# erthward/geonomics

Measured on AMD Instinct MI355X. Metric: individual-timesteps/sec, higher is better.
Workload: dtype u64

## Files before the change

geonomics_amd/csrc/gnx_kernels_demog.hip:

```cpp
#include "gnx_internal.h"
#include <chrono>
#include "gnx_rng.h"
#include "gnx_compact.h"
#include "gnx_half.h"
#include "gnx_xo.h"

#define BIN_BLOCKS 512

__global__ void __launch_bounds__(256)
k_bins(int64_t n, const int32_t* n_dev, const float* x, const float* y, const uint8_t* ghost,
       double inv_hww, int nbx, int nby, int32_t* partials, GnxSetWords sw) {
  extern __shared__ int32_t lds_hist[];
  if (sw.dst && blockIdx.x == 0 && threadIdx.x < 4) sw.dst[threadIdx.x] = sw.v[threadIdx.x];
  if (n_dev) n = *n_dev;
  const int nb = nbx * nby;
  for (int k = threadIdx.x; k < nb; k += blockDim.x) lds_hist[k] = 0;
  __syncthreads();
  const int64_t stride = (int64_t)gridDim.x * blockDim.x;
  for (int64_t i = (int64_t)blockIdx.x * blockDim.x + threadIdx.x; i < n; i += stride) {
    if (ghost && ghost[i]) continue;
    int hx = min(nbx - 1, (int)floor((double)x[i] * inv_hww));
    int hy = min(nby - 1, (int)floor((double)y[i] * inv_hww));
    atomicAdd(&lds_hist[hy * nbx + hx], 1);
  }
  __syncthreads();
  for (int k = threadIdx.x; k < nb; k += blockDim.x) {
    int v = lds_hist[k];
    if (v) atomicAdd(&partials[k], v);
  }
}

__global__ void k_set_words(GnxSetWords sw) {
  if (blockIdx.x == 0 && threadIdx.x < 4) sw.dst[threadIdx.x] = sw.v[threadIdx.x];
}

__global__ void k_bins_global(int64_t n, const float* x, const float* y, const uint8_t* ghost,
                              double inv_hww, int nbx, int nby, int32_t* hist) {
  int64_t i = (int64_t)blockIdx.x * blockDim.x + threadIdx.x;
  if (i >= n) return;
  if (ghost && ghost[i]) return;
  int hx = min(nbx - 1, (int)floor((double)x[i] * inv_hww));
  int hy = min(nby - 1, (int)floor((double)y[i] * inv_hww));
  atomicAdd(&hist[hy * nbx + hx], 1);
}

__global__ void k_nodes(int Jx, int Jy, int nbx, int n_part, const int32_t* partials,
                        const double* areas, double* V) {
  int idx = blockIdx.x * blockDim.x + threadIdx.x;
  if (idx >= Jx * Jy) return;
  int i = idx / Jx, j = idx - i * Jx;
  const int nb = nbx * Jy;
  long long cnt = 0;
  for (int di = -1; di <= 0; ++di)
    for (int dj = -1; dj <= 0; ++dj) {
      int ii = i + di, jj = j + dj;
      if (ii < 0 || jj < 0) continue;
      int b = ii * nbx + jj;
      for (int p = 0; p < n_part; ++p) cnt += partials[(int64_t)p * nb + b];
    }
  V[idx] = (double)cnt / areas[idx];
}

__global__ void k_spline_m(int Jx, int Jy, int along_x, double h, const double* cp,
                           const double* V, double* M) {
// ... 64 lines not shown
  c.hww = h->lat.hww;
  c.inv_hww = 1.0 / h->lat.hww;
  return c;
}

int gnx_l_bins(gnx_state* h, int64_t n, const float* d_x, const float* d_y, const uint8_t* d_ghost,
               int32_t* d_bins, const int32_t* n_dev, const GnxSetWords* sw) {
  const GnxLattice& L = h->lat;
  const int nb = L.nbx * L.nby;
  const int field = (d_bins == h->bins_P) ? 1 : 0;
  if (!h->bins_zeroed[field])
    HIPCHK(hipMemsetAsync(d_bins, 0, (size_t)nb * sizeof(int32_t), h->stream));
  h->bins_zeroed[field] = false;
  if (n > 0) {
    if ((size_t)nb * sizeof(int32_t) <= 48 * 1024) {
      int blocks = (int)std::min<int64_t>(BIN_BLOCKS, std::max<int64_t>(1, (n + 255) / 256));
      hipLaunchKernelGGL(k_bins, dim3(blocks), dim3(256), (size_t)nb * sizeof(int32_t), h->stream,
                         n, n_dev, d_x, d_y, d_ghost, 1.0 / L.hww, L.nbx, L.nby, d_bins,
                         sw ? *sw : GnxSetWords{});
      sw = nullptr;
    } else {
      hipLaunchKernelGGL(k_bins_global, dim3(gnx_grid(n, 256)), dim3(256), 0, h->stream, n, d_x,
                         d_y, d_ghost, 1.0 / L.hww, L.nbx, L.nby, d_bins);
    }
  }
  if (sw)
    hipLaunchKernelGGL(k_set_words, dim3(1), dim3(64), 0, h->stream, *sw);
  HIPCHK(hipGetLastError());
  return 0;
}

__device__ __forceinline__ void spline_line(int J, int64_t base, int64_t stride, double h,
                                            const double* cp, const double* V, double* M) {
  M[base] = 0.0;
  M[base + (int64_t)(J - 1) * stride] = 0.0;
  if (J <= 2) return;
  const double s = 6.0 / (h * h);
  double dprev = 0.0;
  for (int k = 1; k <= J - 2; ++k) {
    double d = s * (V[base + (k - 1) * stride] - 2.0 * V[base + k * stride] +
                    V[base + (k + 1) * stride]);
    double dp = (d - dprev) * cp[k];
    M[base + k * stride] = dp;
    dprev = dp;
  }
  double mnext = dprev;
  for (int k = J - 3; k >= 1; --k) {
    const double m = M[base + k * stride] - cp[k] * mnext;
    M[base + k * stride] = m;
    mnext = m;
  }
}

__device__ __forceinline__ void spline_rows_and_cols(int Jx, int Jy, double hww, const double* cp,
                                                     const double* V, double* Mx, double* My) {
  const int half = blockDim.x / 2;
  if ((int)threadIdx.x < half) {
    for (int line = threadIdx.x; line < Jy; line += half)
      spline_line(Jx, (int64_t)line * Jx, 1, hww, cp, V, Mx);
  } else {
    for (int line = threadIdx.x - half; line < Jx; line += half)
      spline_line(Jy, line, Jx, hww, cp, V, My);
  }
}


__global__ void __launch_bounds__(256)
k_lattice(int Jx, int Jy, int nbx, const int32_t* bins, const double* areas, double hww,
          const double* cp_g, double* C, int32_t* zero_bins, int n_zero,
          unsigned long long* zero_word, int use_lds, int zero_own) {
  extern __shared__ double lat_lds[];
  const int nn = Jx * Jy;
  for (int k = threadIdx.x; k < n_zero; k += blockDim.x) zero_bins[k] = 0;
  if (zero_word && threadIdx.x == 0) *zero_word = 0ull;
  double* W = use_lds ? lat_lds : C;
  double* V = W;
  double* Mx = W + nn;
  double* My = W + 2 * (int64_t)nn;
  double* Mxy = W + 3 * (int64_t)nn;
  const double* cp = cp_g;
  if (use_lds) {
    double* cpl = lat_lds + 4 * (int64_t)nn;
    const int Jm = max(Jx, Jy);
    for (int k = threadIdx.x; k <= Jm; k += blockDim.x) cpl[k] = cp_g[k];
    cp = cpl;
    if (!bins)
      for (int idx = threadIdx.x; idx < nn; idx += blockDim.x) V[idx] = C[idx];
  }
  if (bins) {
    for (int idx = threadIdx.x; idx < nn; idx += blockDim.x) {
      const int i = idx / Jx, j = idx - i * Jx;
      long long cnt = 0;
      for (int di = -1; di <= 0; ++di)
        for (int dj = -1; dj <= 0; ++dj) {
          const int ii = i + di, jj = j + dj;
          if (ii >= 0 && jj >= 0) cnt += bins[ii * nbx + jj];
        }
      V[idx] = (double)cnt / areas[idx];
    }
  }
  __syncthreads();
  if (bins && zero_own)
    for (int k = threadIdx.x; k < nn; k += blockDim.x) const_cast<int32_t*>(bins)[k] = 0;
  spline_rows_and_cols(Jx, Jy, hww, cp, V, Mx, My);
  __syncthreads();
  for (int line = threadIdx.x; line < Jy; line += blockDim.x)
    spline_line(Jx, (int64_t)line * Jx, 1, hww, cp, My, Mxy);
  if (use_lds) {
    __syncthreads();
    for (int idx = threadIdx.x; idx < 4 * nn; idx += blockDim.x) C[idx] = lat_lds[idx];
  }
}

int gnx_l_spline(gnx_state* h, const int32_t* d_bins, GnxSpline* spl,
                 const double* d_nodes_override) {
  return gnx_l_spline_z(h, d_bins, spl, d_nodes_override, false);
}

int gnx_l_spline_z(gnx_state* h, const int32_t* d_bins, GnxSpline* spl,
                   const double* d_nodes_override, bool housekeeping) {
  const GnxLattice& L = h->lat;
  const int64_t nn = (int64_t)L.Jx * L.Jy;
  double* V = spl->c;
  if (d_nodes_override)
    HIPCHK(hipMemcpyAsync(V, d_nodes_override, nn * sizeof(double), hipMemcpyDeviceToDevice,
                          h->stream));
  if (nn <= 65536) {
    int32_t* zb = nullptr;
    int other = -1;
    if (housekeeping && !d_nodes_override) {
      other = (d_bins == h->bins_P) ? 0 : 1;
      zb = other ? h->bins_P : h->bin_partials;
    }
    const size_t lds_bytes = ((size_t)4 * nn + std::max(L.Jx, L.Jy) + 1) * sizeof(double);
    const int use_lds = lds_bytes <= 60 * 1024 ? 1 : 0;
    hipLaunchKernelGGL(k_lattice, dim3(1), dim3(256), use_lds ? lds_bytes : 0, h->stream, L.Jx,
                       L.Jy, L.nbx, d_nodes_override ? nullptr : d_bins, L.areas, L.hww, L.cprime,
                       V, zb, zb ? L.nbx * L.nby : 0,
                       (housekeeping && spl == &h->spl_N) ? h->nmax_bits : nullptr, use_lds, 0);
    if (zb) h->bins_zeroed[other] = true;
    if (housekeeping && spl == &h->spl_N) h->nmax_zeroed = true;
    HIPCHK(hipGetLastError());
    spl->valid = true;
    return 0;
  }
  if (!d_nodes_override)
    hipLaunchKernelGGL(k_nodes, dim3(gnx_grid(nn, 128)), dim3(128), 0, h->stream, L.Jx, L.Jy, L.nbx,
                       1, d_bins, L.areas, V);
  double* Mx = V + nn;
  double* My = V + 2 * nn;
  double* Mxy = V + 3 * nn;
  hipLaunchKernelGGL(k_spline_m, dim3(gnx_grid(L.Jy, 64)), dim3(64), 0, h->stream, L.Jx, L.Jy, 1,
                     L.hww, L.cprime, V, Mx);
  hipLaunchKernelGGL(k_spline_m, dim3(gnx_grid(L.Jx, 64)), dim3(64), 0, h->stream, L.Jx, L.Jy, 0,
                     L.hww, L.cprime, V, My);
  hipLaunchKernelGGL(k_spline_m, dim3(gnx_grid(L.Jy, 64)), dim3(64), 0, h->stream, L.Jx, L.Jy, 1,
                     L.hww, L.cprime, My, Mxy);
  HIPCHK(hipGetLastError());
  spl->valid = true;
  return 0;
}

int gnx_l_density(gnx_state* h, int64_t n, const float* d_x, const float* d_y, GnxSpline* spl,
                  const double* d_nodes_override, const int32_t* n_dev) {
  gnx_time_begin(h);
  int32_t* bins = (spl == &h->spl_P) ? h->bins_P : h->bin_partials;
  if (!d_nodes_override) GNXCHK(gnx_l_bins(h, n, d_x, d_y, nullptr, bins, n_dev));
  GNXCHK(gnx_l_spline_z(h, bins, spl, d_nodes_override, !d_nodes_override));
  gnx_time_end(h, GNX_K_DENSITY, (double)n * 8.0);
  return 0;
}

#define GNX_NMAX_R 8
#define GNX_NMAX_SCAN 12

__host__ __device__ __forceinline__ int gnx_nmax_seg_ints(int Jx) { return 2 * ((Jx + 2) / 2); }

static int gnx_nmax_rows_fit(int Jx, size_t base_doubles) {
  int R = GNX_NMAX_R;
  while (R > 1 && (base_doubles + (size_t)R * 2 * Jx + 256 + gnx_nmax_seg_ints(Jx) / 2) * sizeof(double) >
                      64 * 1024)
    R >>= 1;
  return R;
}
static size_t gnx_nmax_lds_doubles(int Jx, int R) {
  return (size_t)R * 2 * Jx + 256 + gnx_nmax_seg_ints(Jx) / 2;
}
static int gnx_nmax_scan_min() {
  return gnx_env_int("GNX_NMAX_SCAN_ALL", 0) ? 0x7fffffff : GNX_NMAX_SCAN;
}

__device__ __forceinline__ int nmax_seg_of(int cx, double inv_hww, int Jx) {
// ... 37 lines not shown
      const int r = item / (Jx - 1), j = item - r * (Jx - 1);
      if (base + r * row_stride >= H) continue;
      const int lo = seg[j], hi = seg[j + 1] - 1;
      if (lo > hi) continue;
      const double* ab = AB + r * 2 * Jx;
      const double y0 = ab[j], y1 = ab[j + 1], m0 = ab[Jx + j], m1 = ab[Jx + j + 1];
      auto at = [&](int cx) {
        const double tx = (cx + 0.5) * inv_hww - j;
        return spl1(y0, y1, m0, m1, tx, h2_6);
      };
      const double qa = 3.0 * h2_6 * (m1 - m0), qb = 6.0 * h2_6 * m0;
      const double qc = (y1 - y0) - h2_6 * (2.0 * m0 + m1);
      const double disc = qb * qb - 4.0 * qa * qc;
      if (hi - lo < scan_min || !isfinite(disc)) {
        for (int cx = lo; cx <= hi; ++cx) m = fmax(m, at(cx));
        continue;
      }
      m = fmax(m, fmax(at(lo), at(hi)));
      if (disc >= 0.0) {
        const double q = -0.5 * (qb + copysign(sqrt(disc), qb));
        const double root[2] = {q / qa, qc / q};
#pragma unroll
        for (int k = 0; k < 2; ++k) {
          const double cxr = (root[k] + j) * hww - 0.5;
          if (!(cxr > lo - 2.0 && cxr < hi + 2.0)) continue;
          const int k0 = (int)floor(cxr);
          for (int cx = max(k0 - 1, lo); cx <= min(k0 + 2, hi); ++cx) m = fmax(m, at(cx));
        }
      }
    }
  }
  return m;
}

__device__ __forceinline__ void nmax_publish(double m, unsigned long long* out_bits, double* red) {
  red[threadIdx.x] = m;
  __syncthreads();
  for (int s = 128; s > 0; s >>= 1) {
    if (threadIdx.x < s) red[threadIdx.x] = fmax(red[threadIdx.x], red[threadIdx.x + s]);
    __syncthreads();
  }
  if (threadIdx.x == 0) atomicMax(out_bits, (unsigned long long)__double_as_longlong(red[0]));
}

__global__ void __launch_bounds__(256)
k_nmax(SplineC S, int W, int H, unsigned long long* out_bits, int R, int scan_min) {
  extern __shared__ double nmax_lds[];
  double* red = nmax_lds + (size_t)R * 2 * S.Jx;
  const double m = nmax_rows(S.V, S.Jx, S.Jy, S.hww, W, H, blockIdx.x, gridDim.x, nmax_lds,
                             reinterpret_cast<int*>(red + 256), R, scan_min);
  nmax_publish(m, out_bits, red);
}

__global__ void __launch_bounds__(256)
k_lattice_nmax(int Jx, int Jy, int nbx, const int32_t* __restrict__ bins,
               const double* __restrict__ areas, double hww, const double* __restrict__ cp_g,
               double* __restrict__ C, int W, int H, unsigned long long* __restrict__ out_bits,
               int32_t* __restrict__ zero_bins, unsigned long long* __restrict__ zero_word,
               int32_t* __restrict__ binsP, double* __restrict__ CP, GnxPubWords pub, int R, int scan_min) {
  extern __shared__ double lat_lds[];
  const int nn = Jx * Jy;
  const int Jm = max(Jx, Jy);
  const bool isP = binsP != nullptr && blockIdx.x == gridDim.x - 1;
  const int nbN = binsP != nullptr ? (int)gridDim.x - 1 : (int)gridDim.x;
  if (isP) bins = binsP;
  double* V = lat_lds;
  double* Mx = V + nn;
  double* My = V + 2 * nn;
  double* Mxy = V + 3 * nn;
  double* cp = lat_lds + 4 * nn;
  double* AB = cp + Jm + 1;
  double* red = AB + (size_t)R * 2 * Jx;
  int* seg = reinterpret_cast<int*>(red + 256);
  if (blockIdx.x == 0) {
    if (zero_bins)
      for (int k = threadIdx.x; k < nn; k += blockDim.x) zero_bins[k] = 0;
    if (zero_word && threadIdx.x == 0) *zero_word = 0ull;
    if ((int)threadIdx.x < pub.n1)
      __hip_atomic_store(&pub.host1[threadIdx.x], pub.src1[threadIdx.x], __ATOMIC_RELAXED,
                         __HIP_MEMORY_SCOPE_SYSTEM);
    if ((int)threadIdx.x < pub.n2)
      __hip_atomic_store(&pub.host2[threadIdx.x], pub.src2[threadIdx.x], __ATOMIC_RELAXED,
                         __HIP_MEMORY_SCOPE_SYSTEM);
  }
  for (int k = threadIdx.x; k <= Jm; k += blockDim.x) cp[k] = cp_g[k];
  for (int idx = threadIdx.x; idx < nn; idx += blockDim.x) {
    const int i = idx / Jx, j = idx - i * Jx;
    long long cnt = 0;
    for (int di = -1; di <= 0; ++di)
      for (int dj = -1; dj <= 0; ++dj) {
        const int ii = i + di, jj = j + dj;
        if (ii >= 0 && jj >= 0) cnt += bins[ii * nbx + jj];
      }
    V[idx] = (double)cnt / areas[idx];
  }
  __syncthreads();
  spline_rows_and_cols(Jx, Jy, hww, cp, V, Mx, My);
  __syncthreads();
  for (int line = threadIdx.x; line < Jy; line += blockDim.x)
    spline_line(Jx, (int64_t)line * Jx, 1, hww, cp, My, Mxy);
  __syncthreads();
  if (isP) {
    for (int idx = threadIdx.x; idx < 4 * nn; idx += blockDim.x) CP[idx] = lat_lds[idx];
    for (int k = threadIdx.x; k < nn; k += blockDim.x) binsP[k] = 0;
    return;
  }
  if (blockIdx.x == 0)
    for (int idx = threadIdx.x; idx < 4 * nn; idx += blockDim.x) C[idx] = lat_lds[idx];
  const double m = nmax_rows(lat_lds, Jx, Jy, hww, W, H, blockIdx.x, nbN, AB, seg, R, scan_min);
  nmax_publish(m, out_bits, red);
}

struct DemP {
  double R, b, lam, d_min, d_max, K_factor;
  const double* K_over;
  int K_layer, W, H;
  int have_pairs;
};

__device__ __forceinline__ double k_at_cell(const DemP& P, const float* rast, int cx, int cy) {
  if (P.K_over) return P.K_over[(int64_t)cy * P.W + cx];
  return (double)rast[((int64_t)P.K_layer * P.H + cy) * P.W + cx] * P.K_factor;
}

__device__ __forceinline__ double d_at_cell(const DemP& P, double N, double npairs, double K,
                                            double nmax) {
  double dNdt = P.R * (1.0 - (N / K)) * N;
  dNdt = fmax(dNdt, -nmax);
  if (isnan(dNdt) || isinf(dNdt)) dNdt = -nmax;
  double N_b = P.b * P.lam * npairs;
  double N_d = N_b - dNdt;
  double d = N_d / N;
  if (isnan(d)) d = 0.0;
  return fmin(fmax(d, P.d_min), P.d_max);
}

__device__ __forceinline__ double clip_fmax_nan(double v, double lo) {
  return isnan(v) ? v : fmax(v, lo);
}

__global__ void k_raster(int which, SplineC SN, SplineC SP, DemP P, const float* rast,
                         const unsigned long long* nmax_bits, double* out) {
  int64_t c = (int64_t)blockIdx.x * blockDim.x + threadIdx.x;
  if (c >= (int64_t)P.W * P.H) return;
  int cy = (int)(c / P.W), cx = (int)(c - (int64_t)cy * P.W);
  double px = cx + 0.5, py = cy + 0.5;
  double K = k_at_cell(P, rast, cx, cy);
  if (which == GNX_R_K) {
    out[c] = K;
    return;
  }
  double N = fmax(spline_eval(SN, px, py), 0.0);
  if (which == GNX_R_N) {
    out[c] = N;
    return;
  }
  double np_ = P.have_pairs ? fmax(spline_eval(SP, px, py), 0.0) : 0.0;
  if (which == GNX_R_NPAIRS) {
    out[c] = np_;
    return;
  }
  double nmax = __longlong_as_double((long long)*nmax_bits);
  out[c] = d_at_cell(P, N, np_, K, nmax);
// ... 99 lines not shown
  Q.n_delet = (with_selection && h->genomes_assigned) ? h->n_delet : 0;
  Q.n_tl = h->n_tl;
  Q.TW = h->TW;
  return Q;
}

static int launch_nmax(gnx_state* h) {
  if (!h->nmax_zeroed)
    HIPCHK(hipMemsetAsync(h->nmax_bits, 0, sizeof(unsigned long long), h->stream));
  h->nmax_zeroed = false;
  constexpr int GNX_NMAX_BLOCKS = 512;
  const int R = gnx_nmax_rows_fit(h->lat.Jx, 0);
  hipLaunchKernelGGL(k_nmax, dim3(std::min(h->cfg.H, GNX_NMAX_BLOCKS)), dim3(256),
                     gnx_nmax_lds_doubles(h->lat.Jx, R) * sizeof(double), h->stream,
                     make_splinec(h, h->spl_N), h->cfg.W, h->cfg.H, h->nmax_bits, R, gnx_nmax_scan_min());
  h->nmax_cur = h->nmax_bits;
  return 0;
}

constexpr int GNX_LATN_BLOCKS = 256;

bool gnx_fused_bins(const gnx_state* h) {
  const int64_t nn = (int64_t)h->lat.Jx * h->lat.Jy;
  const size_t lds = ((size_t)4 * nn + std::max(h->lat.Jx, h->lat.Jy) + 1 +
                      gnx_nmax_lds_doubles(h->lat.Jx, 1)) * sizeof(double);
  return !h->tiled && !h->tile2_mode && h->fb[0] != nullptr && h->stream3 != nullptr && lds <= 64 * 1024 &&
         (size_t)h->lat.nbx * h->lat.nby * sizeof(int32_t) <= 48 * 1024;
}

int gnx_wait_latP(gnx_state* h) {
  if (h->latP_inflight) {
    HIPCHK(hipStreamWaitEvent(h->stream, h->ev_latP, 0));
    h->latP_inflight = false;
  }
  return 0;
}

int gnx_l_lattice_P_async(gnx_state* h, int64_t n_max) {
  const GnxLattice& L = h->lat;
  const int64_t nn = (int64_t)L.Jx * L.Jy;
  const int nb = L.nbx * L.nby;
  const size_t lds_bytes = ((size_t)4 * nn + std::max(L.Jx, L.Jy) + 1) * sizeof(double);
  GNXCHK(gnx_wait_latP(h));
  HIPCHK(hipEventRecord(h->ev_pairs, h->stream));
  HIPCHK(hipStreamWaitEvent(h->stream3, h->ev_pairs, 0));
  GNXCHK(gnx_bins_adults_launch(h));
  if (!h->fb_zero[2])
    HIPCHK(hipMemsetAsync(h->fb[2], 0, (size_t)nb * sizeof(int32_t), h->stream3));
  const int blocks = (int)std::min<int64_t>(BIN_BLOCKS, std::max<int64_t>(1, (n_max + 255) / 256));
  hipLaunchKernelGGL(k_bins, dim3(blocks), dim3(256), (size_t)nb * sizeof(int32_t), h->stream3,
                     n_max, (const int32_t*)h->cnt_dev, (const float*)h->mid_x,
                     (const float*)h->mid_y, (const uint8_t*)nullptr, 1.0 / L.hww, L.nbx, L.nby,
                     h->fb[2], GnxSetWords{});
  hipLaunchKernelGGL(k_lattice, dim3(1), dim3(256), lds_bytes, h->stream3, L.Jx, L.Jy, L.nbx,
                     (const int32_t*)h->fb[2], L.areas, L.hww, L.cprime, h->spl_P.c,
                     (int32_t*)nullptr, 0, (unsigned long long*)nullptr, 1, 1);
  HIPCHK(hipEventRecord(h->ev_latP, h->stream3));
  HIPCHK(hipGetLastError());
  h->latP_inflight = true;
  h->fb_zero[2] = true;
  h->spl_P.valid = true;
  return 0;
}

int gnx_l_bins_adults_async(gnx_state* h, const float* d_x, const float* d_y, int64_t N) {
  if (!(h->have_sp && gnx_fused_bins(h))) {
    h->fb_adults = false;
    return 0;
  }
  const GnxLattice& L = h->lat;
  const int nb = L.nbx * L.nby;
  const int cur = h->fb_cur;
  if (!h->fb_zero[cur])
    HIPCHK(hipMemsetAsync(h->fb[cur], 0, (size_t)nb * sizeof(int32_t), h->stream));
  h->fbp_x = d_x;
  h->fbp_y = d_y;
  h->fbp_N = N;
  h->fb_pending = true;
  h->fb_zero[cur] = false;
  h->fb_adults = true;
  h->fb_count = N;
  return 0;
}

int gnx_bins_adults_launch(gnx_state* h) {
  if (!h->fb_pending) return 0;
  h->fb_pending = false;
  const GnxLattice& L = h->lat;
  const int nb = L.nbx * L.nby;
  const int64_t N = h->fbp_N;
  const int blocks = (int)std::min<int64_t>(BIN_BLOCKS, std::max<int64_t>(1, (N + 255) / 256));
  hipLaunchKernelGGL(k_bins, dim3(blocks), dim3(256), (size_t)nb * sizeof(int32_t), h->stream3, N,
                     (const int32_t*)nullptr, h->fbp_x, h->fbp_y, (const uint8_t*)nullptr,
                     1.0 / L.hww, L.nbx, L.nby, h->fb[h->fb_cur], GnxSetWords{});
  HIPCHK(hipEventRecord(h->ev_binsN, h->stream3));
  HIPCHK(hipGetLastError());
  h->binsN_inflight = true;
  return 0;
}

void gnx_bins_adults_drop(gnx_state* h) {
  if (h->fb_pending) {
    h->fb_pending = false;
    h->fb_adults = false;
  }
}

int gnx_l_density_N(gnx_state* h) {
  GnxSoA s = h->soa[h->cur];
  if (!(gnx_fused_bins(h) && h->fb_adults && h->fb_count == h->N)) {
    h->fb_adults = false;
    h->nmax_ready = false;
    h->last_N_fused = false;
    return gnx_l_density(h, h->N, s.x, s.y, &h->spl_N, nullptr);
  }
  const GnxLattice& L = h->lat;
  const int64_t nn = (int64_t)L.Jx * L.Jy;
  const size_t lat_doubles = (size_t)4 * nn + std::max(L.Jx, L.Jy) + 1;
  const int nmax_R = gnx_nmax_rows_fit(L.Jx, lat_doubles);
  const size_t lds_bytes = (lat_doubles + gnx_nmax_lds_doubles(L.Jx, nmax_R)) * sizeof(double);
  const int cur = h->fb_cur;
  if (h->fb_pending) {
    HIPCHK(hipEventRecord(h->ev_perm, h->stream));
    HIPCHK(hipStreamWaitEvent(h->stream3, h->ev_perm, 0));
    GNXCHK(gnx_bins_adults_launch(h));
  }
  if (h->binsN_inflight) {
    HIPCHK(hipStreamWaitEvent(h->stream, h->ev_binsN, 0));
    h->binsN_inflight = false;
  }
  gnx_time_begin(h);
  hipLaunchKernelGGL(k_lattice_nmax, dim3(std::max(1, std::min(h->cfg.H, GNX_LATN_BLOCKS))), dim3(256),
                     lds_bytes, h->stream, L.Jx, L.Jy, L.nbx, (const int32_t*)h->fb[cur], L.areas,
                     L.hww, L.cprime, h->spl_N.c, h->cfg.W, h->cfg.H, h->nmax2 + cur,
                     h->fb[cur ^ 1], h->nmax2 + (cur ^ 1), (int32_t*)nullptr, (double*)nullptr,
                     GnxPubWords{}, nmax_R, gnx_nmax_scan_min());
  gnx_time_end(h, GNX_K_DENSITY, (double)h->N * 8.0);
  HIPCHK(hipGetLastError());
  h->spl_N.valid = true;
  h->nmax_cur = h->nmax2 + cur;
  h->nmax_ready = true;
  h->fb_zero[cur] = false;
  h->fb_zero[cur ^ 1] = true;
  h->fb_cur = cur ^ 1;
  h->fb_adults = false;
  h->last_N_fused = true;
  return 0;
}

bool gnx_l_lattices_tiled(gnx_state* h, bool have_pairs, const GnxPubWords& pub) {
  const GnxLattice& L = h->lat;
  const int64_t nn = (int64_t)L.Jx * L.Jy;
  const size_t lat_doubles = (size_t)4 * nn + std::max(L.Jx, L.Jy) + 1;
  const int nmax_R = gnx_nmax_rows_fit(L.Jx, lat_doubles);
  const size_t lds_bytes = (lat_doubles + gnx_nmax_lds_doubles(L.Jx, nmax_R)) * sizeof(double);
  if (lds_bytes > 64 * 1024 || !h->nmax_bits || !h->nmax_zeroed) return false;
  gnx_time_begin(h);
  hipLaunchKernelGGL(k_lattice_nmax,
                     dim3(std::max(1, std::min(h->cfg.H, GNX_LATN_BLOCKS)) + (have_pairs ? 1 : 0)),
                     dim3(256), lds_bytes, h->stream, L.Jx, L.Jy, L.nbx,
                     (const int32_t*)h->bin_partials, L.areas, L.hww, L.cprime, h->spl_N.c, h->cfg.W,
                     h->cfg.H, h->nmax_bits, (int32_t*)nullptr, (unsigned long long*)nullptr,
                     have_pairs ? h->bins_P : (int32_t*)nullptr, h->spl_P.c, pub, nmax_R, gnx_nmax_scan_min());
  gnx_time_end(h, GNX_K_DENSITY, (double)h->N * 8.0);
  h->spl_N.valid = true;
  h->spl_P.valid = have_pairs;
  h->nmax_cur = h->nmax_bits;
  h->nmax_ready = true;
  h->nmax_zeroed = false;
  return true;
}

int gnx_l_death_probs(gnx_state* h, bool with_selection) {
  int64_t N = h->N;
  if (N == 0) return 0;
  SplineC SN = make_splinec(h, h->spl_N), SP = make_splinec(h, h->spl_P);
  GNXCHK(gnx_wait_latP(h));
  gnx_time_begin(h);
  if (!h->nmax_ready) GNXCHK(launch_nmax(h));
  h->nmax_ready = false;
  hipLaunchKernelGGL(k_death_probs, dim3(gnx_grid(N, 256)), dim3(256), 0, h->stream,
                     make_deathp(h, with_selection), make_demp(h), SN, SP, h->soa[h->cur], h->rast,
                     gnx_trait_tab(h), h->delet_s, h->nmax_cur, h->p_death, h->d_cell);
  gnx_time_end(h, GNX_K_DEATH, (double)N * (28.0 + 8.0 * h->cfg.n_traits));
  HIPCHK(hipGetLastError());
  return 0;
}

__global__ void __launch_bounds__(256)
k_alive(int64_t N, const double* p_death, const uint8_t* dead_in, const int64_t* id,
        const uint8_t* ghost, const int32_t* grow, long long step, unsigned long long seed,
        int32_t* alive, int32_t* dead_row, int32_t* cnt, int stride, int64_t xo_first,
        int32_t* zero_jobs, const GnxDD* __restrict__ dd, GnxScanOut scan) {
  __shared__ int lds[16];
  __shared__ int lds2[8];
  const int64_t base = (int64_t)blockIdx.x * GNX_CB;
  if (dd) {
    N = (int64_t)dd->N + dd->B;
    step = dd->step;
    if (xo_first >= 0) xo_first = dd->N;
  }
  if (zero_jobs && blockIdx.x == 0 && threadIdx.x == 0) *zero_jobs = 0;
  bool fa[4], fd[4], fx[4];
#pragma unroll
  for (int r = 0; r < 4; ++r) {
    const int64_t i = base + r * 256 + threadIdx.x;
    fa[r] = fd[r] = fx[r] = false;
    if (i < N) {
      bool dead;
      const bool g = ghost[i] != 0;
      if (g) {
        dead = true;
      } else if (dead_in) {
// ... 915 lines not shown
    h->ord_cur ^= 1;
  } else {
    h->ord_valid = false;
  }
  HIPCHK(hipGetLastError());
  h->mort_wait = true;
  h->mort_xo = xo;
  h->mort_fill = fill;
  h->mort_ord_keep = ord_keep;
  h->mort_has_rows = has_rows;
  h->mort_N = N;
  return 0;
}

int gnx_l_mortality_finish(gnx_state* h, int64_t* deaths_out) {
  *deaths_out = 0;
  if (!h->mort_wait) return 0;
  h->mort_wait = false;
  const bool xo = h->mort_xo, fill = h->mort_fill, ord_keep = h->mort_ord_keep;
  const int has_rows = h->mort_has_rows;
  const int64_t N = h->mort_N;
  {
    const bool ht = gnx_host_times();
    const auto t0 = std::chrono::steady_clock::now();
    HIPCHK(hipEventSynchronize(h->ev_counts));
    if (ht) g_host_wait_s += std::chrono::duration<double>(std::chrono::steady_clock::now() - t0).count();
    gnx_host_mark(2);
  }
  const int64_t survivors = h->h_pin[0];
  const int64_t rows_freed = h->h_pin[1];
  if (xo) {
    const int64_t S = h->h_pin[2];
    h->n_free -= S;
    h->last_xo_births = S;
  }
  if (has_rows) h->n_free += rows_freed;
  *deaths_out = N - h->n_ghost - survivors;
  h->fill_guess = N - survivors;
  h->N = survivors;
  h->n_ghost = 0;
  if (survivors == 0) h->holes = false;
  if (!fill) h->cur ^= 1;
  if (ord_keep) h->ord_n = survivors;
  return 0;
}


int gnx_dd_l_density_N(gnx_state* h, int par, hipStream_t st) {
  const GnxLattice& L = h->lat;
  const int64_t nn = (int64_t)L.Jx * L.Jy;
  const size_t lat_doubles = (size_t)4 * nn + std::max(L.Jx, L.Jy) + 1;
  const int nmax_R = gnx_nmax_rows_fit(L.Jx, lat_doubles);
  const size_t lds_bytes = (lat_doubles + gnx_nmax_lds_doubles(L.Jx, nmax_R)) * sizeof(double);
  hipLaunchKernelGGL(k_lattice_nmax, dim3(std::max(1, std::min(h->cfg.H, GNX_LATN_BLOCKS)) + 1), dim3(256),
                     lds_bytes, st, L.Jx, L.Jy, L.nbx, (const int32_t*)h->fb[par], L.areas, L.hww,
                     L.cprime, h->spl_N.c, h->cfg.W, h->cfg.H, h->nmax2 + par, h->fb[par ^ 1],
                     h->nmax2 + (par ^ 1), h->fb[2], h->spl_P.c, GnxPubWords{}, nmax_R, gnx_nmax_scan_min());
  HIPCHK(hipGetLastError());
  return 0;
}

int gnx_dd_l_death_probs(gnx_state* h, bool with_selection, int par, hipStream_t st) {
  h->spl_N.valid = h->spl_P.valid = true;
  SplineC SN = make_splinec(h, h->spl_N), SP = make_splinec(h, h->spl_P);
  DeathP Q = make_deathp(h, with_selection);
  Q.dd = h->dd;
  hipLaunchKernelGGL(k_death_probs, dim3(gnx_grid(h->cfg.cap_inds, 256)), dim3(256), 0, st, Q,
                     make_demp(h), SN, SP, h->soa[h->cur], h->rast, gnx_trait_tab(h), h->delet_s,
                     (const unsigned long long*)(h->nmax2 + par), h->p_death, h->d_cell);
  HIPCHK(hipGetLastError());
  return 0;
}

int gnx_dd_l_alive(gnx_state* h, bool xo, int buf, hipStream_t st) {
  const gnx_config& c = h->cfg;
  GnxSoA a = h->soa[h->cur];
  const int nb = (int)((c.cap_inds + GNX_CB - 1) / GNX_CB);
  hipLaunchKernelGGL(k_alive, dim3(nb), dim3(256), 0, st, (int64_t)c.cap_inds, h->p_death,
                     (const uint8_t*)nullptr, a.id, a.ghost, a.grow, 0ll, c.seed, h->flag, h->flag2,
                     h->blk_cnt, h->blk_stride, xo ? (int64_t)0 : (int64_t)-1,
                     xo ? h->n_jobs_dev[buf] : (int32_t*)nullptr, (const GnxDD*)h->dd,
                     GnxScanOut{h->blk_off, h->cnt_dev, nullptr, 0, nullptr, h->tickets + 0,
                                h->blk_stride});
  HIPCHK(hipGetLastError());
  return 0;
}

int gnx_dd_l_jobs(gnx_state* h, int buf, hipStream_t st) {
  hipStream_t keep = h->stream;
  h->stream = st;
  h->jobs_self_scan = false;
  gnx_launch_xo_jobs_surv(h, 0, h->flag, h->blk_off, buf);
  h->stream = keep;
  HIPCHK(hipGetLastError());
  return 0;
}

int gnx_dd_l_fill_lists(gnx_state* h, int has_rows, hipStream_t st) {
  const gnx_config& c = h->cfg;
  const int nb = (int)((c.cap_inds + GNX_CB - 1) / GNX_CB);
  hipLaunchKernelGGL(k_fill_lists, dim3(nb), dim3(256), 0, st, (int64_t)c.cap_inds, h->flag, h->flag2,
                     h->blk_off, h->blk_stride, h->cnt_dev, h->soa[h->cur].grow, has_rows,
                     (int32_t*)h->os_ktmp, (int32_t*)h->os_ktmp + c.cap_inds / 2,
                     (int32_t*)h->os_vtmp, h->newslot, h->fill_cnt, (const GnxDD*)h->dd,
                     GnxOrdF{h->ord[h->ord_cur], nullptr, h->flag, h->ord_cnt,
                             GnxScanOut{h->ord_off, nullptr, nullptr, 0, nullptr, h->tickets + 2,
                                        h->blk_stride}, 0, (h->vt_fused && h->id_order == 1) ? 1 : 0});
// ... 92 lines not shown
```

geonomics_amd/csrc/gnx_prim.hip:

```cpp
#include <cstring>
#include <hip/hip_runtime.h>
#include <rocprim/rocprim.hpp>
#include "gnx_internal.h"
#include "gnx_compact.h"

using gnx_sort_config = rocprim::radix_sort_config<rocprim::default_config, rocprim::default_config,
                                                   rocprim::default_config, 8192>;

template <int IPT>
using gnx_onesweep10_t = rocprim::radix_sort_onesweep_config<
    rocprim::kernel_config<1024, IPT>, rocprim::kernel_config<1024, IPT>, 10,
    rocprim::block_radix_rank_algorithm::match>;
template <int IPT>
using gnx_sort_config10_t = rocprim::radix_sort_config<rocprim::default_config, rocprim::default_config,
                                                       gnx_onesweep10_t<IPT>, 8192>;
using gnx_sort_config10 = gnx_sort_config10_t<6>;

int gnx_prim_sort_bytes(size_t n, int bits, size_t* bytes) {
  *bytes = 0;
  HIPCHK(rocprim::radix_sort_pairs<gnx_sort_config>(nullptr, *bytes, (const uint32_t*)nullptr, (uint32_t*)nullptr,
                                   (const int32_t*)nullptr, (int32_t*)nullptr, n, 0, bits,
                                   (hipStream_t)0));
  return 0;
}
// ... 457 lines not shown
    const unsigned int blocks = (unsigned int)((N + 2047) / 2048);
    hipLaunchKernelGGL((gnx_os::k_keys_hist<2>), dim3(blocks), dim3(1024), lds, s, (long long)N,
                       (long long)ord_n, ord, cell32, key, val, (uint32_t*)scratch, places, rb,
                       (long long)N, (1u << end_bit) - 1u, dd);
  } else {
    const unsigned int blocks = (unsigned int)((N + 6143) / 6144);
    hipLaunchKernelGGL((gnx_os::k_keys_hist<6>), dim3(blocks), dim3(1024), lds, s, (long long)N,
                       (long long)ord_n, ord, cell32, key, val, (uint32_t*)scratch, places, rb,
                       (long long)N, (1u << end_bit) - 1u, dd);
  }
  HIPCHK(hipGetLastError());
  return 0;
}
int gnx_os_sort32_ranked(void* scratch, uint32_t* ktmp, int32_t* vtmp, const uint32_t* kin,
                         uint32_t* kout, const int32_t* vin, int32_t* vout, size_t n, int end_bit,
                         hipStream_t s) {
  return gnx_os::passes<uint32_t, GNX_OS_BIG_BS, GNX_OS_BIG_IPT>(
      scratch, ktmp, vtmp, kin, kout, vin, vout, n, end_bit, s, false, nullptr, 0, nullptr);
}
int gnx_os_sort32_gather(void* scratch, uint32_t* ktmp, int32_t* vtmp, uint32_t* kout, int32_t* vout,
                         size_t n, int end_bit, const int32_t* ord, int64_t ord_n,
                         const uint32_t* cell32, hipStream_t s) {
  return gnx_os::passes<uint32_t, GNX_OS_BIG_BS, GNX_OS_BIG_IPT>(
      scratch, ktmp, vtmp, (const uint32_t*)nullptr, kout, (const int32_t*)nullptr, vout, n, end_bit,
      s, true, ord, (long long)ord_n, cell32);
}

size_t gnx_os_words_used64(size_t n, int end_bit) {
  return gnx_os::layout(n, end_bit, GNX_OS_64_BS * GNX_OS_64_IPT).words;
}
int gnx_os_sort64_clean(void* scratch, void* tmp, const uint64_t* kin, uint64_t* kout,
                        const int32_t* vin, int32_t* vout, size_t n, int end_bit, hipStream_t s) {
  uint64_t* ktmp = (uint64_t*)tmp;
  int32_t* vtmp = (int32_t*)(ktmp + n);
  int places, rb;
  gnx_os::digits(end_bit, &places, &rb);
  const unsigned int blocks = (unsigned int)std::min<size_t>((n + 4095) / 4096, 1024);
  hipLaunchKernelGGL((gnx_os::k_hist<uint64_t>), dim3(blocks ? blocks : 1), dim3(512),
                     (size_t)places * (1u << rb) * 4, s, kin, (unsigned int)n, (uint32_t*)scratch,
                     places, rb);
  return gnx_os::passes<uint64_t, GNX_OS_64_BS, GNX_OS_64_IPT>(scratch, ktmp, vtmp, kin, kout, vin,
                                                                vout, n, end_bit, s, false, nullptr,
                                                                0, nullptr);
}

size_t gnx_os_scratch_bytes(size_t n, int end_bit) {
  return gnx_os_words_used(n, end_bit) * sizeof(unsigned int);
}

__global__ void __launch_bounds__(1024)
k_block_scan(int K, int nb, int stride, const int32_t* __restrict__ cnt, int32_t* __restrict__ off,
             int32_t* __restrict__ out, int64_t* __restrict__ host, long long seq,
             const int32_t* __restrict__ extra) {
  __shared__ int wsum[3][16];
  __shared__ int carry_s[3];
  const int tid = threadIdx.x, lane = tid & 63, wave = tid >> 6;
  if (tid < 3) carry_s[tid] = 0;
  __syncthreads();
  for (int b0 = 0; b0 < nb; b0 += 1024) {
    const int b = b0 + tid;
    int v[3], x[3];
#pragma unroll
    for (int k = 0; k < 3; ++k) {
      v[k] = (k < K && b < nb) ? cnt[k * stride + b] : 0;
      x[k] = v[k];
    }
#pragma unroll
    for (int d = 1; d < 64; d <<= 1) {
#pragma unroll
      for (int k = 0; k < 3; ++k) {
        const int y = __shfl_up(x[k], d);
        if (lane >= d) x[k] += y;
      }
    }
    if (lane == 63) {
#pragma unroll
      for (int k = 0; k < 3; ++k) wsum[k][wave] = x[k];
    }
    __syncthreads();
    int tot[3];
#pragma unroll
    for (int k = 0; k < 3; ++k) {
      int woff = 0, t = 0;
      for (int w = 0; w < 16; ++w) {
        const int s = wsum[k][w];
        woff += w < wave ? s : 0;
        t += s;
      }
      tot[k] = t;
      if (k < K && b < nb) off[k * stride + b] = carry_s[k] + woff + x[k] - v[k];
    }
    __syncthreads();
    if (tid < 3) carry_s[tid] += tot[tid];
    __syncthreads();
  }
  if (tid == 0) {
    for (int k = 0; k < 3; ++k) {
      const int total = k < K ? carry_s[k] : 0;
      if (k < K) off[k * stride + nb] = total;
      if (out) out[k] = total;
      if (host) host[k] = total;
    }
    if (host && extra) host[12] = (int64_t)*extra;
    if (host && seq)
      __hip_atomic_store(&host[3], (int64_t)seq, __ATOMIC_RELEASE, __HIP_MEMORY_SCOPE_SYSTEM);
  }
// ... 11 lines not shown
```

Baseline: 2.438 billion.

## Parallelize spline RHS across lattice and batch tridiagonal sweeps; raise wave priority

The spline second-derivative computation is split in two. The stencil right-hand sides for rows and columns are now computed in parallel over every lattice node. Only the Thomas-style forward and backward sweeps stay serial per line, and those load and store in groups of eight so memory latency is exposed less often. Several small latency-bound kernels (bins, lattice, lattice_nmax, block_scan) also raise their wave priority with s_setprio, and k_lattice is templated on LDS use. The adds extra barriers and an extra pass over the planes, and the old path remains reachable through an environment variable.

Result: no change. 2.435 billion (-0.1%).

```diff
diff --git a/geonomics_amd/csrc/gnx_kernels_demog.hip b/geonomics_amd/csrc/gnx_kernels_demog.hip
--- a/geonomics_amd/csrc/gnx_kernels_demog.hip
+++ b/geonomics_amd/csrc/gnx_kernels_demog.hip
@@ -10,6 +10,7 @@
 __global__ void __launch_bounds__(256)
 k_bins(int64_t n, const int32_t* n_dev, const float* x, const float* y, const uint8_t* ghost,
        double inv_hww, int nbx, int nby, int32_t* partials, GnxSetWords sw) {
+  __builtin_amdgcn_s_setprio(3);
   extern __shared__ int32_t lds_hist[];
   if (sw.dst && blockIdx.x == 0 && threadIdx.x < 4) sw.dst[threadIdx.x] = sw.v[threadIdx.x];
   if (n_dev) n = *n_dev;
@@ -180,8 +181,8 @@
   }
 }
 
-__device__ __forceinline__ void spline_rows_and_cols(int Jx, int Jy, double hww, const double* cp,
-                                                     const double* V, double* Mx, double* My) {
+__device__ __forceinline__ void spline_rows_and_cols_plain(int Jx, int Jy, double hww, const double* cp,
+                                                           const double* V, double* Mx, double* My) {
   const int half = blockDim.x / 2;
   if ((int)threadIdx.x < half) {
     for (int line = threadIdx.x; line < Jy; line += half)
@@ -192,22 +193,128 @@
   }
 }
 
-
+#define GNX_SWEEP_GROUP 8
+
+__device__ __forceinline__ void spline_rhs_rows(int Jx, int Jy, double s, const double* __restrict__ V,
+                                                double* __restrict__ M) {
+  const int nn = Jx * Jy;
+  for (int idx = threadIdx.x; idx < nn; idx += blockDim.x) {
+    const int k = idx % Jx;
+    double d = 0.0;
+    if (k > 0 && k < Jx - 1) d = s * (V[idx - 1] - 2.0 * V[idx] + V[idx + 1]);
+    M[idx] = d;
+  }
+}
+
+__device__ __forceinline__ void spline_rhs_cols(int Jx, int Jy, double s, const double* __restrict__ V,
+                                                double* __restrict__ M) {
+  const int nn = Jx * Jy;
+  for (int idx = threadIdx.x; idx < nn; idx += blockDim.x) {
+    const int k = idx / Jx;
+    double d = 0.0;
+    if (k > 0 && k < Jy - 1) d = s * (V[idx - Jx] - 2.0 * V[idx] + V[idx + Jx]);
+    M[idx] = d;
+  }
+}
+
+__device__ __forceinline__ void spline_chain(int J, int stride, const double* __restrict__ cp,
+                                             double* __restrict__ M) {
+  if (J <= 2) return;
+  constexpr int G = GNX_SWEEP_GROUP;
+  double dprev = 0.0;
+  int k = 1;
+  for (; k + G - 1 <= J - 2; k += G) {
+    double d[G], c[G];
+#pragma unroll
+    for (int u = 0; u < G; ++u) {
+      d[u] = M[(k + u) * stride];
+      c[u] = cp[k + u];
+    }
+#pragma unroll
+    for (int u = 0; u < G; ++u) {
+      d[u] = (d[u] - dprev) * c[u];
+      dprev = d[u];
+    }
+#pragma unroll
+    for (int u = 0; u < G; ++u) M[(k + u) * stride] = d[u];
+  }
+  for (; k <= J - 2; ++k) {
+    const double dp = (M[k * stride] - dprev) * cp[k];
+    M[k * stride] = dp;
+    dprev = dp;
+  }
+  double mnext = dprev;
+  k = J - 3;
+  for (; k - (G - 1) >= 1; k -= G) {
+    double d[G], c[G];
+#pragma unroll
+    for (int u = 0; u < G; ++u) {
+      d[u] = M[(k - u) * stride];
+      c[u] = cp[k - u];
+    }
+#pragma unroll
+    for (int u = 0; u < G; ++u) {
+      d[u] = d[u] - c[u] * mnext;
+      mnext = d[u];
+    }
+#pragma unroll
+    for (int u = 0; u < G; ++u) M[(k - u) * stride] = d[u];
+  }
+  for (; k >= 1; --k) {
+    const double m = M[k * stride] - cp[k] * mnext;
+    M[k * stride] = m;
+    mnext = m;
+  }
+}
+
+template <bool PLAIN>
+__device__ __forceinline__ void spline_planes(int Jx, int Jy, double hww, const double* __restrict__ cp,
+                                              double* __restrict__ V, double* __restrict__ Mx,
+                                              double* __restrict__ My, double* __restrict__ Mxy) {
+  if (PLAIN) {
+    spline_rows_and_cols_plain(Jx, Jy, hww, cp, V, Mx, My);
+    __syncthreads();
+    for (int line = threadIdx.x; line < Jy; line += blockDim.x)
+      spline_line(Jx, (int64_t)line * Jx, 1, hww, cp, My, Mxy);
+    return;
+  }
+  const double s = 6.0 / (hww * hww);
+  const int half = blockDim.x / 2;
+  spline_rhs_rows(Jx, Jy, s, V, Mx);
+  spline_rhs_cols(Jx, Jy, s, V, My);
+  __syncthreads();
+  if ((int)threadIdx.x < half) {
+    for (int line = threadIdx.x; line < Jy; line += half) spline_chain(Jx, 1, cp, Mx + line * Jx);
+  } else {
+    for (int line = threadIdx.x - half; line < Jx; line += half) spline_chain(Jy, Jx, cp, My + line);
+  }
+  __syncthreads();
+  spline_rhs_rows(Jx, Jy, s, My, Mxy);
+  __syncthreads();
+  for (int line = threadIdx.x; line < Jy; line += blockDim.x) spline_chain(Jx, 1, cp, Mxy + line * Jx);
+}
+
+static bool gnx_lattice_plain() { return gnx_env_int("GNX_LATTICE_PLAIN", 0) != 0; }
+
+
+template <bool USE_LDS, bool PLAIN>
 __global__ void __launch_bounds__(256)
-k_lattice(int Jx, int Jy, int nbx, const int32_t* bins, const double* areas, double hww,
-          const double* cp_g, double* C, int32_t* zero_bins, int n_zero,
-          unsigned long long* zero_word, int use_lds, int zero_own) {
+k_lattice(int Jx, int Jy, int nbx, const int32_t* __restrict__ bins, const double* __restrict__ areas,
+          double hww, const double* __restrict__ cp_g, double* __restrict__ C,
+          int32_t* __restrict__ zero_bins, int n_zero, unsigned long long* __restrict__ zero_word,
+          int zero_own) {
+  __builtin_amdgcn_s_setprio(3);
   extern __shared__ double lat_lds[];
   const int nn = Jx * Jy;
   for (int k = threadIdx.x; k < n_zero; k += blockDim.x) zero_bins[k] = 0;
   if (zero_word && threadIdx.x == 0) *zero_word = 0ull;
-  double* W = use_lds ? lat_lds : C;
+  double* W = USE_LDS ? lat_lds : C;
   double* V = W;
   double* Mx = W + nn;
   double* My = W + 2 * (int64_t)nn;
   double* Mxy = W + 3 * (int64_t)nn;
   const double* cp = cp_g;
-  if (use_lds) {
+  if (USE_LDS) {
     double* cpl = lat_lds + 4 * (int64_t)nn;
     const int Jm = max(Jx, Jy);
     for (int k = threadIdx.x; k <= Jm; k += blockDim.x) cpl[k] = cp_g[k];
@@ -230,14 +337,20 @@
   __syncthreads();
   if (bins && zero_own)
     for (int k = threadIdx.x; k < nn; k += blockDim.x) const_cast<int32_t*>(bins)[k] = 0;
-  spline_rows_and_cols(Jx, Jy, hww, cp, V, Mx, My);
-  __syncthreads();
-  for (int line = threadIdx.x; line < Jy; line += blockDim.x)
-    spline_line(Jx, (int64_t)line * Jx, 1, hww, cp, My, Mxy);
-  if (use_lds) {
+  spline_planes<PLAIN>(Jx, Jy, hww, cp, V, Mx, My, Mxy);
+  if (USE_LDS) {
     __syncthreads();
     for (int idx = threadIdx.x; idx < 4 * nn; idx += blockDim.x) C[idx] = lat_lds[idx];
   }
+}
+
+template <typename... A>
+static void launch_lattice(bool use_lds, size_t lds_bytes, hipStream_t st, A... a) {
+  const bool plain = gnx_lattice_plain();
+  if (use_lds && plain) hipLaunchKernelGGL((k_lattice<true, true>), dim3(1), dim3(256), lds_bytes, st, a...);
+  else if (use_lds) hipLaunchKernelGGL((k_lattice<true, false>), dim3(1), dim3(256), lds_bytes, st, a...);
+  else if (plain) hipLaunchKernelGGL((k_lattice<false, true>), dim3(1), dim3(256), 0, st, a...);
+  else hipLaunchKernelGGL((k_lattice<false, false>), dim3(1), dim3(256), 0, st, a...);
 }
 
 int gnx_l_spline(gnx_state* h, const int32_t* d_bins, GnxSpline* spl,
@@ -262,10 +375,10 @@
     }
     const size_t lds_bytes = ((size_t)4 * nn + std::max(L.Jx, L.Jy) + 1) * sizeof(double);
     const int use_lds = lds_bytes <= 60 * 1024 ? 1 : 0;
-    hipLaunchKernelGGL(k_lattice, dim3(1), dim3(256), use_lds ? lds_bytes : 0, h->stream, L.Jx,
-                       L.Jy, L.nbx, d_nodes_override ? nullptr : d_bins, L.areas, L.hww, L.cprime,
-                       V, zb, zb ? L.nbx * L.nby : 0,
-                       (housekeeping && spl == &h->spl_N) ? h->nmax_bits : nullptr, use_lds, 0);
+    launch_lattice(use_lds != 0, lds_bytes, h->stream, L.Jx, L.Jy, L.nbx,
+                   d_nodes_override ? (const int32_t*)nullptr : d_bins, (const double*)L.areas, L.hww,
+                   (const double*)L.cprime, V, zb, zb ? L.nbx * L.nby : 0,
+                   (housekeeping && spl == &h->spl_N) ? h->nmax_bits : (unsigned long long*)nullptr, 0);
     if (zb) h->bins_zeroed[other] = true;
     if (housekeeping && spl == &h->spl_N) h->nmax_zeroed = true;
     HIPCHK(hipGetLastError());
@@ -409,12 +522,14 @@
   nmax_publish(m, out_bits, red);
 }
 
+template <bool PLAIN>
 __global__ void __launch_bounds__(256)
 k_lattice_nmax(int Jx, int Jy, int nbx, const int32_t* __restrict__ bins,
                const double* __restrict__ areas, double hww, const double* __restrict__ cp_g,
                double* __restrict__ C, int W, int H, unsigned long long* __restrict__ out_bits,
                int32_t* __restrict__ zero_bins, unsigned long long* __restrict__ zero_word,
                int32_t* __restrict__ binsP, double* __restrict__ CP, GnxPubWords pub, int R, int scan_min) {
+  __builtin_amdgcn_s_setprio(3);
   extern __shared__ double lat_lds[];
   const int nn = Jx * Jy;
   const int Jm = max(Jx, Jy);
@@ -452,10 +567,7 @@
     V[idx] = (double)cnt / areas[idx];
   }
   __syncthreads();
-  spline_rows_and_cols(Jx, Jy, hww, cp, V, Mx, My);
-  __syncthreads();
-  for (int line = threadIdx.x; line < Jy; line += blockDim.x)
-    spline_line(Jx, (int64_t)line * Jx, 1, hww, cp, My, Mxy);
+  spline_planes<PLAIN>(Jx, Jy, hww, cp, V, Mx, My, Mxy);
   __syncthreads();
   if (isP) {
     for (int idx = threadIdx.x; idx < 4 * nn; idx += blockDim.x) CP[idx] = lat_lds[idx];
@@ -466,6 +578,12 @@
     for (int idx = threadIdx.x; idx < 4 * nn; idx += blockDim.x) C[idx] = lat_lds[idx];
   const double m = nmax_rows(lat_lds, Jx, Jy, hww, W, H, blockIdx.x, nbN, AB, seg, R, scan_min);
   nmax_publish(m, out_bits, red);
+}
+
+template <typename... A>
+static void launch_lattice_nmax(int blocks, size_t lds_bytes, hipStream_t st, A... a) {
+  if (gnx_lattice_plain()) hipLaunchKernelGGL(k_lattice_nmax<true>, dim3(blocks), dim3(256), lds_bytes, st, a...);
+  else hipLaunchKernelGGL(k_lattice_nmax<false>, dim3(blocks), dim3(256), lds_bytes, st, a...);
 }
 
 struct DemP {
@@ -671,9 +789,9 @@
                      n_max, (const int32_t*)h->cnt_dev, (const float*)h->mid_x,
                      (const float*)h->mid_y, (const uint8_t*)nullptr, 1.0 / L.hww, L.nbx, L.nby,
                      h->fb[2], GnxSetWords{});
-  hipLaunchKernelGGL(k_lattice, dim3(1), dim3(256), lds_bytes, h->stream3, L.Jx, L.Jy, L.nbx,
-                     (const int32_t*)h->fb[2], L.areas, L.hww, L.cprime, h->spl_P.c,
-                     (int32_t*)nullptr, 0, (unsigned long long*)nullptr, 1, 1);
+  launch_lattice(true, lds_bytes, h->stream3, L.Jx, L.Jy, L.nbx, (const int32_t*)h->fb[2],
+                 (const double*)L.areas, L.hww, (const double*)L.cprime, h->spl_P.c, (int32_t*)nullptr, 0,
+                 (unsigned long long*)nullptr, 1);
   HIPCHK(hipEventRecord(h->ev_latP, h->stream3));
   HIPCHK(hipGetLastError());
   h->latP_inflight = true;
@@ -749,7 +867,7 @@
     h->binsN_inflight = false;
   }
   gnx_time_begin(h);
-  hipLaunchKernelGGL(k_lattice_nmax, dim3(std::max(1, std::min(h->cfg.H, GNX_LATN_BLOCKS))), dim3(256),
+  launch_lattice_nmax(std::max(1, std::min(h->cfg.H, GNX_LATN_BLOCKS)),
                      lds_bytes, h->stream, L.Jx, L.Jy, L.nbx, (const int32_t*)h->fb[cur], L.areas,
                      L.hww, L.cprime, h->spl_N.c, h->cfg.W, h->cfg.H, h->nmax2 + cur,
                      h->fb[cur ^ 1], h->nmax2 + (cur ^ 1), (int32_t*)nullptr, (double*)nullptr,
@@ -775,9 +893,8 @@
   const size_t lds_bytes = (lat_doubles + gnx_nmax_lds_doubles(L.Jx, nmax_R)) * sizeof(double);
   if (lds_bytes > 64 * 1024 || !h->nmax_bits || !h->nmax_zeroed) return false;
   gnx_time_begin(h);
-  hipLaunchKernelGGL(k_lattice_nmax,
-                     dim3(std::max(1, std::min(h->cfg.H, GNX_LATN_BLOCKS)) + (have_pairs ? 1 : 0)),
-                     dim3(256), lds_bytes, h->stream, L.Jx, L.Jy, L.nbx,
+  launch_lattice_nmax(std::max(1, std::min(h->cfg.H, GNX_LATN_BLOCKS)) + (have_pairs ? 1 : 0),
+                     lds_bytes, h->stream, L.Jx, L.Jy, L.nbx,
                      (const int32_t*)h->bin_partials, L.areas, L.hww, L.cprime, h->spl_N.c, h->cfg.W,
                      h->cfg.H, h->nmax_bits, (int32_t*)nullptr, (unsigned long long*)nullptr,
                      have_pairs ? h->bins_P : (int32_t*)nullptr, h->spl_P.c, pub, nmax_R, gnx_nmax_scan_min());
@@ -1799,7 +1916,7 @@
   const size_t lat_doubles = (size_t)4 * nn + std::max(L.Jx, L.Jy) + 1;
   const int nmax_R = gnx_nmax_rows_fit(L.Jx, lat_doubles);
   const size_t lds_bytes = (lat_doubles + gnx_nmax_lds_doubles(L.Jx, nmax_R)) * sizeof(double);
-  hipLaunchKernelGGL(k_lattice_nmax, dim3(std::max(1, std::min(h->cfg.H, GNX_LATN_BLOCKS)) + 1), dim3(256),
+  launch_lattice_nmax(std::max(1, std::min(h->cfg.H, GNX_LATN_BLOCKS)) + 1,
                      lds_bytes, st, L.Jx, L.Jy, L.nbx, (const int32_t*)h->fb[par], L.areas, L.hww,
                      L.cprime, h->spl_N.c, h->cfg.W, h->cfg.H, h->nmax2 + par, h->fb[par ^ 1],
                      h->nmax2 + (par ^ 1), h->fb[2], h->spl_P.c, GnxPubWords{}, nmax_R, gnx_nmax_scan_min());
diff --git a/geonomics_amd/csrc/gnx_prim.hip b/geonomics_amd/csrc/gnx_prim.hip
--- a/geonomics_amd/csrc/gnx_prim.hip
+++ b/geonomics_amd/csrc/gnx_prim.hip
@@ -533,6 +533,7 @@
 k_block_scan(int K, int nb, int stride, const int32_t* __restrict__ cnt, int32_t* __restrict__ off,
              int32_t* __restrict__ out, int64_t* __restrict__ host, long long seq,
              const int32_t* __restrict__ extra) {
+  __builtin_amdgcn_s_setprio(3);
   __shared__ int wsum[3][16];
   __shared__ int carry_s[3];
   const int tid = threadIdx.x, lane = tid & 63, wave = tid >> 6;
```
